# san-soucie/gdrf

Measured on AMD Instinct MI355X. Metric: ELBO steps/sec (+ achieved HBM GB/s on K_nm) at N=1e6,M=512,K=10,V=50, higher is better.
Workload: dtype f32; 1 GPU; configs[3] at 1 GPU(s): N=1000000 synthetic 2-D lattice (1000x1000), V=50, K=10, M=512 (32x16 grid inducing points), rbf kernel, Adam lr=1e-3, Trace_ELBO, 1 particle, jitter=1e-06, observations sharded over ranks; N=1000000, M=512, K=10, V=50, D=2, rows_per_rank=1000000, jitter_level=2, stores_T=False, mfma_mode=f16x3

## Files before the change

### gdrf_amd/csrc/api.hip

```cpp
#include "../../include/gdrf_hip.h"
#include "common.h"
#include "gemm_nt.h"
#include "gemm_tn.h"
#include "gemm_split.h"
#include "gemm_tn_topics.h"
#include "gemm_tn_topics1.h"
#include "kernels_mm.h"
#include "kernels_n.h"
#include "predict.h"
#include "predict_mc.h"
#include "predict_info.h"
#include "foldin.h"
#include "sample_counts.h"
#include "predict_cov.h"
#include "select_batch.h"
#include "rows_lds.h"
#include "rows_mfma.h"
#include "rows_vstream.h"
#include "rows_csr.h"
#include "hyper_tn.h"
#include "optim.h"

#include <algorithm>
#include <cmath>
// ... 831 lines not shown
        constexpr int lds4 = 8 * SplitCfg<SP>::IMG * 2 + 8 * GDRF_TILE * 4;
        HIPCHK(hipFuncSetAttribute((const void*)fwd_t_split_q4_kernel<SP>, hipFuncAttributeMaxDynamicSharedMemorySize, lds4));
        hipLaunchKernelGGL(fwd_t_split_q4_kernel<SP>, dim3((unsigned)(8 * K * rt8)), dim3(1024), lds4, s, a);
      } else {
        constexpr int lds2 = 6 * SplitCfg<SP>::IMG * 2;
        HIPCHK(hipFuncSetAttribute((const void*)fwd_t_split_cc_kernel<SP>, hipFuncAttributeMaxDynamicSharedMemorySize, lds2));
        hipLaunchKernelGGL(fwd_t_split_cc_kernel<SP>, dim3((unsigned)(8 * K * rt8)), dim3(512), lds2, s, a);
      }
      LAUNCHCHK("fwd_t_split");
      return 0;
    } else {
      return fail(-1, "fwd_t_split", "float arrays only");
    }
  }

  template <class SP>
  static int tn_split(gdrf_ctx* c, const float* B, const float* scale, int64_t scale_bs, int64_t n, int64_t rps, int sym, float* slab,
                      int nbatch, int ns, int ntiles, int sidx_b, int sidx_b_stride, hipStream_t s, const void* Ah = nullptr, int sidx_a = -1) {
    if constexpr (std::is_same<T, float>::value) {
      using E = typename SP::E;
      TNSplitArgs<SP> a{(const E*)(Ah ? Ah : c->Wh), (int64_t)c->ncap * c->Mp, c->Mp, B, c->Mp, scale, scale_bs, n, rps, c->Mp, sym, slab, nbatch, ns,
                        (const float*)c->ssc, sidx_a >= 0 ? sidx_a : SplitLay{c->K}.w(), sidx_b, sidx_b_stride};
      constexpr int lds = 3 * SP::NP * 32 * 128 * 2;
      HIPCHK(hipFuncSetAttribute((const void*)gemm_tn_split_kernel<SP>, hipFuncAttributeMaxDynamicSharedMemorySize, lds));
      hipLaunchKernelGGL(gemm_tn_split_kernel<SP>, dim3((unsigned)(ntiles * nbatch * ns)), dim3(256), lds, s, a);
      return 0;
    } else {
      return fail(-1, "tn_split", "float arrays only");
    }
  }

  template <class SP>
  static int wbar_split(gdrf_ctx* c, int64_t n, const T* U, int64_t rtiles, hipStream_t s) {
    if constexpr (std::is_same<T, float>::value) {
      using E = typename SP::E;
      const int Mp = c->Mp, K = c->K;
      const SplitLay SL{K};
      const int64_t nb = (int64_t)K * Mp * Mp;
      hipLaunchKernelGGL(split_blocked_kernel<SP>, dim3((unsigned)((nb / 4 + 255) / 256)), dim3(256), 0, s, (const float*)c->Bm, nb, Mp, Mp, (E*)c->Bh, nb,
                         (const float*)c->ssc + SL.b(0));
      BwdWbarSplitArgs<SP> a{(const float*)c->W, (const E*)c->Wh, (int64_t)c->ncap * Mp, n, c->M, Mp, K, (const E*)c->Bh, nb,
                             (const float*)c->vbar, (const float*)c->locbar, c->ldk, (const float*)c->asum, (const float*)U, (float*)c->Wbar,
                             (const float*)c->ssc, c->smx + SL.mx_wbar()};
      const size_t grp = SplitCfg<SP>::LDS_BYTES + (((size_t)K * GDRF_TILE * sizeof(float) + 15) & ~(size_t)15);
      const int nct_ = (Mp + GDRF_TILE - 1) / GDRF_TILE;
      if (K >= 2 && 2 * grp <= 160 * 1024) {
        const int64_t pairs = (rtiles + 1) / 2;
        const size_t tabb = ((size_t)K * GDRF_TILE * sizeof(float) + 15) & ~(size_t)15;
        const size_t lds_cc = 6 * (size_t)SplitCfg<SP>::IMG * 2 + 2 * tabb;
        if (std::is_same<SP, SplitF16>::value && K >= 2 && (Mp % 64) == 0 && 8 * (size_t)SplitCfg<SP>::IMG * 2 + 2 * tabb <= 160 * 1024) {
          if constexpr (std::is_same<SP, SplitF16>::value) {
            const size_t lds64 = 8 * (size_t)SplitCfg<SP>::IMG * 2 + 2 * tabb;
            const int nkb = Mp / 64;
            int nslice = 1;
            if (pairs * nct_ <= 32 && nkb >= 2) nslice = std::min(nkb, 8);
            if ((size_t)nslice * round_up(n, 256) * Mp > (size_t)c->nsplit_cap * (K + 1) * Mp * Mp) nslice = 1;
            if (nslice > 1) { a.slab = (float*)c->slab; a.slab_stride = (int64_t)round_up(n, 256) * Mp; a.nslice = nslice; }
            c->forms[GDRF_FORM_WBAR] = 6; c->forms[GDRF_FORM_WBAR_NSLICE] = nslice;
            HIPCHK(hipFuncSetAttribute((const void*)bwd_wbar_f16_k64_kernel, hipFuncAttributeMaxDynamicSharedMemorySize, (int)lds64));
            hipLaunchKernelGGL(bwd_wbar_f16_k64_kernel, dim3((unsigned)round_up(pairs * nct_, 8), (unsigned)nslice), dim3(512), lds64, s, a);
            if (nslice > 1) {
              const int64_t n4 = n * Mp / 4;
              hipLaunchKernelGGL(wbar_slab_sum_kernel, dim3((unsigned)((n4 + 255) / 256)), dim3(256), 0, s, (const float*)a.slab, a.slab_stride, nslice, n4,
                                 (float*)c->Wbar, a.wbar_max);
            }
          }
        } else if (lds_cc <= 160 * 1024) {
          HIPCHK(hipFuncSetAttribute((const void*)bwd_wbar_split_cc_kernel<SP>, hipFuncAttributeMaxDynamicSharedMemorySize, (int)lds_cc));
          hipLaunchKernelGGL((bwd_wbar_split_cc_kernel<SP>), dim3((unsigned)round_up(pairs * nct_, 8)), dim3(512), lds_cc, s, a);
          c->forms[GDRF_FORM_WBAR] = 5; c->forms[GDRF_FORM_WBAR_NSLICE] = 1;
        } else {
          const size_t lds = std::max<size_t>(2 * grp, 8 * 32 * 68 * sizeof(float));
          HIPCHK(hipFuncSetAttribute((const void*)bwd_wbar_split_kernel<SP, 2>, hipFuncAttributeMaxDynamicSharedMemorySize, (int)lds));
          hipLaunchKernelGGL((bwd_wbar_split_kernel<SP, 2>), dim3((unsigned)round_up(pairs * nct_, 8)), dim3(512), lds, s, a);
          c->forms[GDRF_FORM_WBAR] = 4; c->forms[GDRF_FORM_WBAR_NSLICE] = 1;
        }
      } else {
        if (grp > 160 * 1024) return fail(-1, "wbar_split", "too many topics for the LDS scale table");
        const size_t lds = std::max<size_t>(grp, 4 * 32 * 68 * sizeof(float));
        HIPCHK(hipFuncSetAttribute((const void*)bwd_wbar_split_kernel<SP, 1>, hipFuncAttributeMaxDynamicSharedMemorySize, (int)lds));
        hipLaunchKernelGGL((bwd_wbar_split_kernel<SP, 1>), dim3((unsigned)round_up(rtiles * nct_, 8)), dim3(256), lds, s, a);
        c->forms[GDRF_FORM_WBAR] = 3; c->forms[GDRF_FORM_WBAR_NSLICE] = 1;
      }
      LAUNCHCHK("wbar_split");
      return 0;
    } else {
      return fail(-1, "wbar_split", "float arrays only");
    }
  }

  static int knm_solve(gdrf_ctx* c, const T* X, int64_t n, hipStream_t s) {
    ScopedTimer tm(c, 1, s);
    const int VE = Vec16<TS>::N;
    const int vpr = (c->Mp + VE - 1) / VE, rpp = vpr <= 256 ? 256 / vpr : 1;
    int64_t blocks = (n + 4 * rpp - 1) / (4 * rpp);
    const int64_t kcap = 256 * 64;
    if (blocks > kcap) blocks = kcap;
    if (blocks < 1) blocks = 1;
    if constexpr (sizeof(TS) == 8) {
      if (c->kind == 0 && vpr <= 256) {
        auto go = [&](auto kern) {
          hipLaunchKernelGGL(kern, dim3((unsigned)blocks), dim3(256), 0, s, X, n, (const double*)Q(c->Zs), c->M, c->D, c->hyp, (double*)Q(c->Knm),
                             (int64_t)c->Mp);
        };
        if (ard_fwd(c)) { if (c->D <= 2) go(knm_rbf_f64_kernel<T, 2, true, true>); else go(knm_rbf_f64_kernel<T, GDRF_DMAX, true, true>); }
        else { if (c->D <= 2) go(knm_rbf_f64_kernel<T, 2>); else go(knm_rbf_f64_kernel<T, GDRF_DMAX>); }
// ... 1377 lines not shown
```

### gdrf_amd/csrc/gemm_split.h

```cpp
#pragma once
#include "common.h"
#include "gemm_nt.h"
#include "kernels_mm.h"

namespace gdrf {

typedef __bf16 bf16x8 __attribute__((ext_vector_type(8)));
typedef __bf16 bf16x4 __attribute__((ext_vector_type(4)));
typedef _Float16 f16x8 __attribute__((ext_vector_type(8)));
typedef _Float16 f16x4 __attribute__((ext_vector_type(4)));
typedef float f32x4 __attribute__((ext_vector_type(4)));
typedef uint32_t u32x4 __attribute__((ext_vector_type(4)));

struct SplitBf16 {
  using E = __bf16; using V8 = bf16x8; using V4 = bf16x4;
  static constexpr int NP = 3, NPROD = 6, ID = 1;
  static __device__ __forceinline__ constexpr int pa(int t) { constexpr int v[6] = {0, 1, 2, 0, 1, 0}; return v[t]; }
  static __device__ __forceinline__ constexpr int pb(int t) { constexpr int v[6] = {2, 1, 0, 1, 0, 0}; return v[t]; }
  static __device__ __forceinline__ f32x4 mma(V8 a, V8 b, f32x4 c) { return __builtin_amdgcn_mfma_f32_16x16x32_bf16(a, b, c, 0, 0, 0); }
  static __device__ __forceinline__ void split(float x, E (&p)[NP]) {
    p[0] = (__bf16)x;
    const float r1 = x - (float)p[0];
    p[1] = (__bf16)r1;
    p[2] = (__bf16)(r1 - (float)p[1]);
  }
};
struct SplitF16 {
  using E = _Float16; using V8 = f16x8; using V4 = f16x4;
  static constexpr int NP = 2, NPROD = 3, ID = 2;
  static __device__ __forceinline__ constexpr int pa(int t) { constexpr int v[3] = {0, 1, 0}; return v[t]; }
  static __device__ __forceinline__ constexpr int pb(int t) { constexpr int v[3] = {1, 0, 0}; return v[t]; }
  static __device__ __forceinline__ f32x4 mma(V8 a, V8 b, f32x4 c) { return __builtin_amdgcn_mfma_f32_16x16x32_f16(a, b, c, 0, 0, 0); }
  static __device__ __forceinline__ void split(float y, E (&p)[NP]) {
    p[0] = (_Float16)y;
    p[1] = (_Float16)(y - (float)p[0]);
  }
};

struct SplitLay {
  int K;
  __host__ __device__ int w() const { return 0; }
  __host__ __device__ int wbar() const { return 2; }
  __host__ __device__ int b(int k) const { return 4 + 2 * k; }
  __host__ __device__ int st(int k) const { return 4 + 2 * K + 2 * k; }
  __host__ __device__ int v(int k) const { return 4 + 4 * K + 2 * k; }
  __host__ __device__ int dk() const { return 4 + 6 * K; }
  __host__ __device__ int nfloats() const { return 6 + 6 * K; }
  __host__ __device__ int mx_wbar() const { return 0; }
  __host__ __device__ int mx_b(int k) const { return 1 + k; }
  __host__ __device__ int mx_st(int k) const { return 1 + K + k; }
  __host__ __device__ int mx_v(int k) const { return 1 + 2 * K + k; }
  __host__ __device__ int nmax() const { return 1 + 3 * K; }
};
// ... 9 lines not shown
__global__ void split_scales_kernel(int f16, const Hyper* __restrict__ h, const unsigned* __restrict__ mx, float* __restrict__ sc, int K, int what) {
  const SplitLay L{K};
  auto put = [&](int idx, float s) { sc[idx] = s; sc[idx + 1] = 1.0f / s; };
  const int t = threadIdx.x;
  if ((what & SPLIT_SC_W) && t == 0)
    put(L.w(), f16 ? split_pow2_scale(sqrtf((float)h->var), 13) : 1.0f);
  if ((what & SPLIT_SC_W) && t == 0) put(L.dk(), f16 ? split_pow2_scale(0.75f * (float)h->var, 15) : 1.0f);
  if ((what & SPLIT_SC_WBAR) && t == 0) put(L.wbar(), f16 ? split_pow2_scale(__uint_as_float(mx[L.mx_wbar()]), 15) : 1.0f);
  for (int k = t; k < K; k += blockDim.x) {
    if (what & SPLIT_SC_BST) {
      put(L.b(k), f16 ? split_pow2_scale(__uint_as_float(mx[L.mx_b(k)]), 15) : 1.0f);
      put(L.st(k), f16 ? split_pow2_scale(__uint_as_float(mx[L.mx_st(k)]), 15) : 1.0f);
    }
    if (what & SPLIT_SC_V) put(L.v(k), f16 ? split_pow2_scale(__uint_as_float(mx[L.mx_v(k)]) * sqrtf((float)h->var), 13) : 1.0f);
  }
}
__device__ __forceinline__ void wave_max_publish(unsigned* mx, float m) {
#pragma unroll
  for (int o = 32; o > 0; o >>= 1) m = fmaxf(m, __shfl_xor(m, o, 64));
  if ((threadIdx.x & 63) == 0 && m > 0) atomicMax(mx, __float_as_uint(m));
}

__global__ __launch_bounds__(256) void absmax_batched_kernel(const float* __restrict__ x, int64_t n, int64_t ld, unsigned* __restrict__ mx) {
  const int b = blockIdx.y;
  float m = 0;
  const f32x4* p = reinterpret_cast<const f32x4*>(x + (int64_t)b * ld);
  for (int64_t i = (int64_t)blockIdx.x * blockDim.x + threadIdx.x; i < (n >> 2); i += (int64_t)gridDim.x * blockDim.x) {
    const f32x4 v = p[i];
    m = fmaxf(fmaxf(m, fmaxf(fabsf(v[0]), fabsf(v[1]))), fmaxf(fabsf(v[2]), fabsf(v[3])));
  }
  if (blockIdx.x == 0 && threadIdx.x < (n & 3)) m = fmaxf(m, fabsf(x[(int64_t)b * ld + (n & ~(int64_t)3) + threadIdx.x]));
  wave_max_publish(mx + b, m);
}

template <class SP> struct SplitCfg {
  static constexpr int BK = 32;
  static constexpr int LDH = BK;
  static constexpr int PIECE = GDRF_TILE * LDH;
  static constexpr int IMG = SP::NP * PIECE;
  static constexpr int LDS_BYTES = 2 * IMG * 2;
};
__device__ __forceinline__ int split_swz(int row) { return (row & 8) ? 3 : 0; }
__device__ __forceinline__ int split_off(int row, int k) { return row * 32 + (((k >> 3) ^ split_swz(row)) << 3) + (k & 7); }

__device__ __forceinline__ void glds16_asm(const void* gsrc, unsigned lds_dst) {
  asm volatile("s_mov_b32 m0, %1\n\ts_nop 0\n\tglobal_load_lds_dwordx4 %0, off" : : "v"(gsrc), "s"(lds_dst) : "memory");
}
__device__ __forceinline__ void glds16_asm_s(const void* sbase, unsigned voff, unsigned lds_dst) {
  asm volatile("s_mov_b32 m0, %2\n\ts_nop 0\n\tglobal_load_lds_dwordx4 %0, %1" : : "v"(voff), "s"(sbase), "s"(lds_dst) : "memory");
}
__device__ __forceinline__ unsigned lds_addr(const void* p) {
  return (unsigned)(uintptr_t)(__attribute__((address_space(3))) const void*)p;
}


struct SplitLane {
  int tid, lane, wave;
  int wr, wc;
  int lr, lg;
  __device__ __forceinline__ SplitLane() {
    tid = threadIdx.x & 255; lane = tid & 63; wave = tid >> 6;
    wr = wave >> 1; wc = wave & 1; lr = lane & 15; lg = lane >> 4;
  }
  __device__ __forceinline__ int wave_u() const { return __builtin_amdgcn_readfirstlane(wave); }
  __device__ __forceinline__ int frag() const { return lr * 32 + ((lg ^ split_swz(lr)) << 3); }
  __device__ __forceinline__ int drow() const { return lane >> 2; }
  __device__ __forceinline__ int dq() const { return ((lane & 3) ^ split_swz(drow())) * 8; }
};

__device__ __forceinline__ void split_zero(f32x4 (&acc)[4][4]) {
#pragma unroll
  for (int a = 0; a < 4; ++a)
#pragma unroll
    for (int b = 0; b < 4; ++b) acc[a][b] = f32x4{0, 0, 0, 0};
}
template <class SP> __device__ __forceinline__ typename SP::V8 split_frag(const typename SP::E* img, int p, int row0, int frag) {
  return *reinterpret_cast<const typename SP::V8*>(img + p * SplitCfg<SP>::PIECE + row0 * 32 + frag);
}
template <class SP> __device__ __forceinline__ void split_frags(typename SP::V8 (&f)[SP::NP], const typename SP::E* img, int row0, int frag) {
#pragma unroll
  for (int p = 0; p < SP::NP; ++p) f[p] = split_frag<SP>(img, p, row0, frag);
}
template <class SP, bool FIRST>
__device__ __forceinline__ void split_products(f32x4 (&P)[4], const typename SP::V8 (&fa)[4][SP::NP], const typename SP::V8 (&fb)[SP::NP]) {
#pragma unroll
  for (int t = 0; t < SP::NPROD; ++t)
#pragma unroll
    for (int a = 0; a < 4; ++a) P[a] = SP::mma(fa[a][SP::pa(t)], fb[SP::pb(t)], (FIRST && t == 0) ? f32x4{0, 0, 0, 0} : P[a]);
}
__device__ __forceinline__ void split_row_scales(f32x4 (&s4)[4], const float* sc_row, const SplitLane& L) {
#pragma unroll
  for (int a = 0; a < 4; ++a) s4[a] = *reinterpret_cast<const f32x4*>(sc_row + L.wr * 64 + a * 16 + L.lg * 4);
}
__device__ __forceinline__ void split_scaled_acc(f32x4 (&acc)[4][4], int b, const f32x4 (&s4)[4], const f32x4 (&P)[4]) {
#pragma unroll
  for (int a = 0; a < 4; ++a)
#pragma unroll
    for (int r = 0; r < 4; ++r) acc[a][b][r] += s4[a][r] * P[a][r];
}
__device__ __forceinline__ void split_phase_end() {
  asm volatile("s_waitcnt vmcnt(0)" ::: "memory");
  asm volatile("s_waitcnt lgkmcnt(0)" ::: "memory");
  gdrf_raw_barrier();
}


// ... 465 lines not shown
      const int64_t mc = m < g.nrows ? m : 0;
      const int nc = n < Mp ? n : 0;
      wv[h][i] = *reinterpret_cast<const f32x4*>(g.W + mc * Mp + nc);
      as2v[h][i] = first_slice ? 2.0f * g.asum[mc] : 0.0f;
    }
  const int wr = L.wr, wc = L.wc, lr = L.lr, lg = L.lg;
  for (int kb = 0; kb < (first_slice ? K : 0); kb += 16) {
    float av[4][4], bv[4][4];
#pragma unroll
    for (int it = 0; it < 4; ++it) {
      const int k = kb + 4 * it + lg, kc = k < K ? k : 0;
#pragma unroll
      for (int a = 0; a < 4; ++a) {
        const int64_t row = m0 + wr * 64 + a * 16 + lr;
        const float v = g.locbar[(int64_t)kc * g.ldk + (row < g.nrows ? row : 0)];
        av[it][a] = (k < K && row < g.nrows) ? v : 0.0f;
      }
#pragma unroll
      for (int b = 0; b < 4; ++b) {
        const int col = n0 + wc * 64 + b * 16 + lr;
        const float v = g.U[(int64_t)kc * g.M + (col < g.M ? col : 0)];
        bv[it][b] = (k < K && col < g.M) ? v : 0.0f;
      }
    }
#pragma unroll
    for (int it = 0; it < 4; ++it) {
      if (kb + 4 * it < K) {
#pragma unroll
        for (int a = 0; a < 4; ++a)
#pragma unroll
          for (int b = 0; b < 4; ++b) acc[a][b] = __builtin_amdgcn_mfma_f32_16x16x4f32(av[it][a], bv[it][b], acc[a][b], 0, 0, 0);
      }
    }
  }
  __syncthreads();
  float wmax = 0.0f;
  float* tile = wbar_tile(smem, gp, L);
#pragma unroll
  for (int h = 0; h < 2; ++h) {
    wbar_tile_put(tile, acc, h, L);
#pragma unroll
    for (int i = 0; i < 8; ++i) {
      const int64_t m = m0 + L.wr * 64 + h * 32 + ((L.lane >> 4) + 4 * i);
      const int n = n0 + L.wc * 64 + (L.lane & 15) * 4;
      const f32x4 t = wbar_tile_get(tile, i, L);
      if (m < g.nrows && n < Mp) wbar_seg_store(out_base + m * Mp + n, t, as2v[h][i], wv[h][i], wmax);
    }
    asm volatile("s_waitcnt lgkmcnt(0)" ::: "memory");
  }
  if (g.wbar_max && g.nslice == 1) wave_max_publish(g.wbar_max, wmax);
}


__global__ __launch_bounds__(256) void wbar_slab_sum_kernel(const float* __restrict__ slab, int64_t slab_stride, int nslice, int64_t n4 ,
                                                           float* __restrict__ Wbar, unsigned* __restrict__ wbar_max) {
  const int64_t i = (int64_t)blockIdx.x * blockDim.x + threadIdx.x;
  float wmax = 0.0f;
  if (i < n4) {
    f32x4 acc = *reinterpret_cast<const f32x4*>(slab + 4 * i);
    for (int sl = 1; sl < nslice; ++sl) {
      const f32x4 t = *reinterpret_cast<const f32x4*>(slab + (int64_t)sl * slab_stride + 4 * i);
#pragma unroll
      for (int e = 0; e < 4; ++e) acc[e] += t[e];
    }
    *reinterpret_cast<f32x4*>(Wbar + 4 * i) = acc;
#pragma unroll
    for (int e = 0; e < 4; ++e) wmax = fmaxf(wmax, fabsf(acc[e]));
  }
  if (wbar_max) wave_max_publish(wbar_max, wmax);
}

template <class SP> struct FwdTSplitArgs {
  const typename SP::E* Wh; int64_t w_stride; int64_t nrows; int Mp, K;
  int KG; int rt8;
  const typename SP::E* STh; int64_t piece_stride;
  float* tt; int64_t ldt;
  const float* sc;
};

template <class SP> __device__ __forceinline__ void fwd_t_map_block(const FwdTSplitArgs<SP>& g, int64_t& rt0, int& bz) {
  const unsigned xcd = blockIdx.x & 7u, idx = blockIdx.x >> 3;
  const unsigned per_group = (unsigned)g.KG * (unsigned)g.rt8;
  const int grp = (int)(idx / per_group);
  const unsigned rem = idx - (unsigned)grp * per_group;
  const int kg = min(g.KG, g.K - grp * g.KG);
  rt0 = 2 * ((int64_t)(rem / (unsigned)kg) * 8 + xcd);
  bz = grp * g.KG + (int)(rem % (unsigned)kg);
}
__device__ __forceinline__ bool fwd_t_col_ok(int ct, int b, int Mp, const SplitLane& L) { return ct * GDRF_TILE + L.wc * 64 + b * 16 + L.lr < Mp; }
__device__ __forceinline__ float fwd_t_sq(float x, bool cok) { return cok ? x * x : 0.0f; }
template <class SP> __device__ __forceinline__ void fwd_t_store_tt(const FwdTSplitArgs<SP>& g, int bz, int64_t m0, int tid, float v) {
  const int64_t m = m0 + tid;
  const SplitLay SL{g.K};
  const float un = g.sc[SL.w() + 1] * g.sc[SL.st(bz) + 1];
  if (m < g.nrows) g.tt[(int64_t)bz * g.ldt + m] = v * (un * un);
}


template <class SP>
__global__ __launch_bounds__(512, 2) void fwd_t_split_cc_kernel(FwdTSplitArgs<SP> g) {
  using CF = SplitCfg<SP>;
  using E = typename SP::E;
  using V8 = typename SP::V8;
  constexpr int NP = SP::NP;
  extern __shared__ __attribute__((aligned(16))) char smem[];
  constexpr int IMG = CF::IMG;
// ... 422 lines not shown
```

### gdrf_amd/csrc/gemm_tn_topics1.h

```cpp
#pragma once
#include <utility>
#include "gemm_tn_topics.h"

namespace gdrf {

template <int... Is, class F> __device__ __forceinline__ void static_for_impl(std::integer_sequence<int, Is...>, F&& f) {
  (f(std::integral_constant<int, Is>{}), ...);
}
template <int N, class F> __device__ __forceinline__ void static_for(F&& f) { static_for_impl(std::make_integer_sequence<int, N>{}, f); }

constexpr int TN1_CH = 64;
constexpr int TN1_XBLK = 1056;
constexpr int TN1_X_BYTES = 16 * TN1_XBLK;
constexpr int TN1_VROWS = 12;
constexpr int TN1_V_BYTES = TN1_VROWS * TN1_CH * 4;
constexpr int TN1_NBUF = 3;

__device__ __forceinline__ void glds4_asm(const void* gsrc, unsigned lds_dst) {
  asm volatile("s_mov_b32 m0, %1\n\ts_nop 0\n\tglobal_load_lds_dword %0, off" : : "v"(gsrc), "s"(lds_dst) : "memory");
}

__device__ __forceinline__ void glds4_asm_s(const void* sbase, unsigned voff, unsigned lds_dst) {
  asm volatile("s_mov_b32 m0, %2\n\ts_nop 0\n\tglobal_load_lds_dword %0, %1" : : "v"(voff), "s"(sbase), "s"(lds_dst) : "memory");
}

__global__ void tn1_scale_rows_kernel(const float* __restrict__ vbar, int64_t ldk, int64_t nrows, float* __restrict__ vs, int64_t lds,
                                      const float* __restrict__ sc, int sidx_v) {
  const int k = blockIdx.y;
  const float scale = sc[sidx_v + 2 * k];
  for (int64_t n = (int64_t)blockIdx.x * blockDim.x + threadIdx.x; n < lds; n += (int64_t)gridDim.x * blockDim.x)
    vs[(int64_t)k * lds + n] = n < nrows ? vbar[(int64_t)k * ldk + n] * scale : 0.0f;
}

constexpr int TN2_A_BYTES = 2 * 2 * 32 * 128 * 2;
constexpr int TN2_BUF = TN2_A_BYTES + TN1_X_BYTES + TN1_V_BYTES;
constexpr int TN2_DMA_PER_CHUNK = 15;
constexpr int tn2_lds_bytes() { return TN1_NBUF * TN2_BUF; }

__host__ __device__ inline int tn2_ntiles_half(int ncols) {
  const int nI = (ncols + 127) / 128, nJ = (ncols + 63) / 64;
  int t = 0;
  for (int I = 0; I < nI; ++I) t += (2 * I + 1 < nJ) ? 1 : 0;
  return t;
}
template <int AMIN>
__global__ __launch_bounds__(256, 1) void tn_topics_w2_kernel(TNTopicsArgs g) {
  using E = _Float16;
  using V8 = f16x8;
  using V4 = f16x4;
  constexpr int KT = TNT_KT, PIECE = 32 * 128, KA = 8;
  static_assert(KT == 10, "register plan below is for 10 topics");
  extern __shared__ __attribute__((aligned(16))) char smem[];
  const int tid = threadIdx.x, lane = tid & 63;
  const int w = __builtin_amdgcn_readfirstlane(tid >> 6);
  const int lr = lane & 15, lg = lane >> 4;
  const int kgroups = (g.K + KT - 1) / KT;
  const unsigned units = (unsigned)(g.ntiles * kgroups), bid = blockIdx.x;
  unsigned u; int sp;
  if ((g.nsplit & 7) == 0) { const unsigned idx = bid >> 3; sp = (int)(idx / units) * 8 + (int)(bid & 7u); u = idx % units; }
  else { sp = (int)(bid / units); u = bid % units; }
  const int tile = (int)(u % (unsigned)g.ntiles), gk = (int)(u / (unsigned)g.ntiles);
  int I = 0, J = tile;
// ... 217 lines not shown
```

### gdrf_amd/engine.py

```python
from __future__ import annotations

import contextlib
import ctypes as C
import math
from typing import Dict, Optional

import torch

from . import _lib
from .data import check_counts, is_sparse_counts

KERNEL_IDS = {"rbf": 0, "matern52": 1, "matern32": 2, "exponential": 3, "rationalquadratic": 4, "periodic": 5, "product": 6}
PRODUCT_KINDS = {"rbf": 0, "periodic": 5}
OPT_MODES = {"adam": 0, "adamw": 1, "clippedadam": 2}
OPT_RULES = {"adam": 0, "adamw": 1, "clippedadam": 2, "adamax": 3, "rmsprop": 4, "adagrad": 5, "adadelta": 6, "asgd": 7, "rprop": 8,
             "adagradrmsprop": 9}
OPT_CLIP_NORM, OPT_CLIP_VALUE, OPT_MOMENTUM, OPT_CENTERED = 1, 2, 4, 8

_WS_IDS = dict(W=0, Wbar=1, q=2, loc=3, tt=4, vbar=5, locbar=6, asum=7, Kuu=8, L=9, Linv=10, S=11, B=12, phi=13,
               mu=14, LinvT=15, ST=16, Knm=17, g_locbar=18)


def _stream_ptr(device) -> int:
    return torch.cuda.current_stream(device).cuda_stream
# ... 362 lines not shown
            fi = torch.finfo(self.dtype)
            y = self.Z.clamp(min=fi.tiny, max=1.0 - fi.eps)
            self.view("inducing_unc").copy_(y.log() - (-y).log1p())

    def refresh_inducing(self):
        if self.learn_inducing:
            torch.sigmoid(self.view("inducing_unc"), out=self.Z)

    def set_dirichlet(self, alpha: torch.Tensor):
        a = alpha.detach().to("cpu", torch.float64).contiguous()
        assert a.shape == (self.K, self.V)
        arr = (C.c_double * (self.K * self.V))(*a.flatten().tolist())
        _lib.check(self.lib.gdrf_set_dirichlet(self.ctx, arr), "gdrf_set_dirichlet")

    def workspace(self, name: str, n_rows: Optional[int] = None) -> torch.Tensor:
        ptr, cnt = C.c_void_p(), C.c_int64()
        _lib.check(self.lib.gdrf_ws_ptr(self.ctx, _WS_IDS[name], C.byref(ptr), C.byref(cnt)), "gdrf_ws_ptr")
        esz = self.lib.gdrf_ws_elem_size(self.ctx, _WS_IDS[name])
        flat = torch.empty(cnt.value, dtype=torch.float32 if esz == 4 else torch.float64, device=self.device)
        _lib.check(self.lib.gdrf_ws_copy(self.ctx, _WS_IDS[name], flat.data_ptr(), cnt.value, _stream_ptr(self.device)),
                   "gdrf_ws_copy")
        torch.cuda.synchronize(self.device)
        Mp = (self.M + 31) // 32 * 32
        ldk = (self.n_cap + 3) // 4 * 4
        n = self.n_cap if n_rows is None else n_rows
        if name in ("W", "Wbar", "Knm"):
            return flat.view(self.n_cap, Mp)[:n, :self.M].clone()
        if name in ("q", "asum"):
            return flat[:n].clone()
        if name in ("loc", "tt", "vbar", "locbar", "mu"):
            return flat.view(self.K, ldk)[:, :n].clone()
        if name in ("Kuu", "L", "Linv", "LinvT"):
            return flat.view(Mp, Mp)[:self.M, :self.M].clone()
        if name in ("S", "B", "ST"):
            return flat.view(self.K, Mp, Mp)[:, :self.M, :self.M].clone()
        if name == "phi":
            return flat.view(self.K, self.V).clone()
        raise KeyError(name)

    TIMING_SLOTS = ("probe", "k_nm", "transforms", "fwd_w", "loc", "fwd_t", "elbo_rows", "bwd_wbar", "bwd_knm",
                    "tn_sym", "tn_gt", "slab_reduce", "ubar", "step_finish", "adam", "factorize")

    def set_timing(self, enable: bool):
        _lib.check(self.lib.gdrf_set_timing(self.ctx, 1 if enable else 0), "gdrf_set_timing")

    def get_timing(self) -> Dict[str, Dict[str, float]]:
        n = len(self.TIMING_SLOTS)
        ms, cnt = (C.c_double * n)(), (C.c_int64 * n)()
        _lib.check(self.lib.gdrf_get_timing(self.ctx, ms, cnt, n), "gdrf_get_timing")
        return {name: dict(ms=ms[i], count=cnt[i]) for i, name in enumerate(self.TIMING_SLOTS)}

    FORM_SLOTS = ("wbar", "wbar_nslice", "a_k", "a_k_kgroups", "fwd_t", "fwd_t_kg", "loc", "ubar_q4", "rows", "rows_kt", "rows_vt", "gt",
                  "hyper", "predict", "predict_nb")
    FORM_NAMES = dict(wbar=("gemm_nt", "gemm_nt_t", "split<1>", "split<2>", "split_cc", "k64"), a_k=("gemm_tn", "tn_split", "tn_topics", "w2"),
                      fwd_t=("gemm_nt", "q4", "cc"), loc=("rows", "gemm_nt", "gemm_nt_wide"), rows=("mfma", "thread", "streamed"),
                      gt=("gemm_tn", "tn_split"), hyper=("f64", "tn"), predict=("mfma", "rows_lds", "rows_mem", "rows_bigk", "streamed"))

    def last_forms(self) -> Dict[str, object]:
        n = len(self.FORM_SLOTS)
        arr = (C.c_int * n)()
        _lib.check(self.lib.gdrf_last_forms(self.ctx, arr, n), "gdrf_last_forms")
        out = {}
        for slot, v in zip(self.FORM_SLOTS, arr):
            if v:
                out[slot] = self.FORM_NAMES[slot][v - 1] if slot in self.FORM_NAMES else v
        return out

    def _chk_rows(self, xs: torch.Tensor, ws: Optional[torch.Tensor] = None):
        if xs.device != self.device or xs.dtype != self.dtype or not xs.is_contiguous() or xs.dim() != 2 or xs.shape[1] != self.D:
            raise ValueError(f"xs must be a contiguous ({'n'},{self.D}) {self.dtype} tensor on {self.device}")
        if ws is not None and is_sparse_counts(ws):
            check_counts(ws, xs.shape[0], self.V, self.device)
        elif ws is not None:
            if ws.device != self.device or ws.dtype != torch.int32 or not ws.is_contiguous() or ws.shape != (xs.shape[0], self.V):
                raise ValueError(f"ws must be a contiguous (n,{self.V}) int32 tensor on {self.device}")

    def _counts_ptr(self, ws: Optional[torch.Tensor]):
        if ws is None or not is_sparse_counts(ws):
            if self._csr_bound:
                _lib.check(self.lib.gdrf_bind_counts_csr(self.ctx, None, None, None, 0, 0, None, None), "gdrf_bind_counts_csr")
                self._csr_bound = False
            return None if ws is None else ws.data_ptr()
        c = self._csr_cache
        if c is None or c[0] is not ws or c[1] != ws._version:
            crow = ws.crow_indices().to(torch.int64).contiguous()
            col = ws.col_indices().to(torch.int32).contiguous()
            val = ws.values().contiguous()
            order = torch.sort(col, stable=True)
            cperm = order.indices.to(torch.int64).contiguous()
            ccol = torch.searchsorted(order.values, torch.arange(self.V + 1, dtype=torch.int32, device=self.device)).to(torch.int64).contiguous()
            c = self._csr_cache = (ws, ws._version, (crow, col, val, ccol, cperm))
            self._csr_bound = False
        if not self._csr_bound:
            crow, col, val, ccol, cperm = c[2]
            _lib.check(self.lib.gdrf_bind_counts_csr(self.ctx, crow.data_ptr(), col.data_ptr(), val.data_ptr(), ws.shape[0], col.numel(),
                                                     ccol.data_ptr(), cperm.data_ptr()), "gdrf_bind_counts_csr")
            self._csr_bound = True
        return None

    def knm(self, xs: torch.Tensor) -> torch.Tensor:
        self._chk_rows(xs)
        out = torch.empty(xs.shape[0], self.M, dtype=self.dtype, device=self.device)
        self.knm_into(xs, out)
        return out

    def knm_into(self, xs: torch.Tensor, out: torch.Tensor):
        _lib.check(self.lib.gdrf_knm(self.ctx, xs.data_ptr(), xs.shape[0], self.Z.data_ptr(), self.params.data_ptr(),
# ... 519 lines not shown
```

Before: 24.37 steps/s.

## Add hand-scheduled AGPR-resident f16-split Wbar backward kernel for large row counts

Adds a new Wbar backward kernel, used when there are many row tiles and K is at most 16. It holds W fragments and B tiles in AGPRs through inline assembly and interleaves MFMA, global loads, LDS DMA and scale reads on a fixed static schedule. It uses one wave per column half, 256 threads and a single block per CU, and folds the rank-K locbar·U correction in afterwards with fp32 MFMA. The goal is to hide memory latency and raise MFMA utilization compared with the k64 kernel, at the cost of very fragile hand-tuned code: clobbering every AGPR, hard-coded vmcnt counts and low occupancy. The static_for helper moves into a shared header.

After: 24.85 steps/s (median of 6 runs). 1.02x the previous value.

```diff
diff --git a/gdrf_amd/csrc/api.hip b/gdrf_amd/csrc/api.hip
--- a/gdrf_amd/csrc/api.hip
+++ b/gdrf_amd/csrc/api.hip
@@ -907,6 +907,19 @@
           if constexpr (std::is_same<SP, SplitF16>::value) {
             const size_t lds64 = 8 * (size_t)SplitCfg<SP>::IMG * 2 + 2 * tabb;
             const int nkb = Mp / 64;
+            if (pairs * nct_ > 32 && K <= 16) {
+              const size_t lds_w1 = 8 * (size_t)SplitCfg<SP>::IMG * 2 + 2 * (size_t)(K + 1) * GDRF_TILE * sizeof(float);
+              const dim3 grid((unsigned)round_up(pairs * nct_, 8));
+              auto launch = [&](auto kern) {
+                HIPCHK(hipFuncSetAttribute((const void*)kern, hipFuncAttributeMaxDynamicSharedMemorySize, (int)lds_w1));
+                hipLaunchKernelGGL(kern, grid, dim3(256), lds_w1, s, a);
+                return 0;
+              };
+              if (int rc = K >= 8 ? launch(bwd_wbar_f16_w1_kernel<2>) : (K >= 4 ? launch(bwd_wbar_f16_w1_kernel<4>) : launch(bwd_wbar_f16_w1_kernel<8>))) return rc;
+              c->forms[GDRF_FORM_WBAR] = 7; c->forms[GDRF_FORM_WBAR_NSLICE] = 1;
+              LAUNCHCHK("wbar_split");
+              return 0;
+            }
             int nslice = 1;
             if (pairs * nct_ <= 32 && nkb >= 2) nslice = std::min(nkb, 8);
             if ((size_t)nslice * round_up(n, 256) * Mp > (size_t)c->nsplit_cap * (K + 1) * Mp * Mp) nslice = 1;
diff --git a/gdrf_amd/csrc/gemm_split.h b/gdrf_amd/csrc/gemm_split.h
--- a/gdrf_amd/csrc/gemm_split.h
+++ b/gdrf_amd/csrc/gemm_split.h
@@ -1,4 +1,5 @@
 #pragma once
+#include <utility>
 #include "common.h"
 #include "gemm_nt.h"
 #include "kernels_mm.h"
@@ -114,6 +115,11 @@
 __device__ __forceinline__ unsigned lds_addr(const void* p) {
   return (unsigned)(uintptr_t)(__attribute__((address_space(3))) const void*)p;
 }
+
+template <int... Is, class F> __device__ __forceinline__ void static_for_impl(std::integer_sequence<int, Is...>, F&& f) {
+  (f(std::integral_constant<int, Is>{}), ...);
+}
+template <int N, class F> __device__ __forceinline__ void static_for(F&& f) { static_for_impl(std::make_integer_sequence<int, N>{}, f); }
 
 
 struct SplitLane {
@@ -685,6 +691,255 @@
 }
 
 
+#define GDRF_A10(p) "a" p "0", "a" p "1", "a" p "2", "a" p "3", "a" p "4", "a" p "5", "a" p "6", "a" p "7", "a" p "8", "a" p "9"
+#define GDRF_A100(p) GDRF_A10(p "0"), GDRF_A10(p "1"), GDRF_A10(p "2"), GDRF_A10(p "3"), GDRF_A10(p "4"), GDRF_A10(p "5"), GDRF_A10(p "6"), \
+                     GDRF_A10(p "7"), GDRF_A10(p "8"), GDRF_A10(p "9")
+#define GDRF_ALL_AGPRS "a0", "a1", "a2", "a3", "a4", "a5", "a6", "a7", "a8", "a9", GDRF_A10("1"), GDRF_A10("2"), GDRF_A10("3"), GDRF_A10("4"), \
+                       GDRF_A10("5"), GDRF_A10("6"), GDRF_A10("7"), GDRF_A10("8"), GDRF_A10("9"), GDRF_A100("1"), GDRF_A10("20"), GDRF_A10("21"), \
+                       GDRF_A10("22"), GDRF_A10("23"), GDRF_A10("24"), "a250", "a251", "a252", "a253", "a254", "a255"
+constexpr int wb1_wreg(int ks, int a, int p) { return ((ks * 8 + a) * 2 + p) * 4; }
+constexpr int wb1_breg(int h, int ks, int b, int p) { return 128 + (((h * 2 + ks) * 4 + b) * 2 + p) * 4; }
+template <int WA, int BA, bool ZERO> __device__ __forceinline__ void wb1_mfma(f32x4& P) {
+  if constexpr (ZERO) asm volatile("v_mfma_f32_16x16x32_f16 %0, a[%c1:%c2], a[%c3:%c4], 0" : "=v"(P) : "i"(WA), "i"(WA + 3), "i"(BA), "i"(BA + 3));
+  else asm volatile("v_mfma_f32_16x16x32_f16 %0, a[%c1:%c2], a[%c3:%c4], %0" : "+v"(P) : "i"(WA), "i"(WA + 3), "i"(BA), "i"(BA + 3));
+}
+template <int REG, int OFF> __device__ __forceinline__ void wb1_gload(const void* sbase, unsigned voff) {
+  asm volatile("global_load_dwordx4 a[%c2:%c3], %0, %1 offset:%c4" : : "v"(voff), "s"(sbase), "i"(REG), "i"(REG + 3), "i"(OFF) : "memory", GDRF_ALL_AGPRS);
+}
+template <int REG, int OFF> __device__ __forceinline__ void wb1_ldsread(unsigned addr) {
+  asm volatile("ds_read_b128 a[%c1:%c2], %0 offset:%c3" : : "v"(addr), "i"(REG), "i"(REG + 3), "i"(OFF) : "memory", GDRF_ALL_AGPRS);
+}
+template <int R0> __device__ __forceinline__ void wb1_update2(float& c0, float& c1, const f32x4& s, const f32x4& p) {
+  asm volatile("v_fmac_f32 %0, %1, %2" : "+v"(c0) : "v"(s[R0]), "v"(p[R0]));
+  asm volatile("v_fmac_f32 %0, %1, %2" : "+v"(c1) : "v"(s[R0 + 1]), "v"(p[R0 + 1]));
+}
+template <int N> __device__ __forceinline__ void wb1_vmcnt() { asm volatile("s_waitcnt vmcnt(%0)" : : "n"(N) : "memory"); }
+
+template <int R>
+__global__ __launch_bounds__(256, 1) void bwd_wbar_f16_w1_kernel(BwdWbarSplitArgs<SplitF16> g) {
+  using SP = SplitF16;
+  using CF = SplitCfg<SP>;
+  using E = typename SP::E;
+  static_assert(R == 2 || R == 4 || R == 8, "16 requests per block in K >= 16 / R phases");
+  constexpr int PIECE = CF::PIECE;
+  constexpr int WIMG = 4 * PIECE * 2;
+  extern __shared__ __attribute__((aligned(16))) char smem[];
+  SplitLane L;
+  const int w = L.wave_u(), gp = w >> 1, wc = w & 1;
+  L.wc = wc;
+  const int K = g.K, Mp = g.Mp;
+  const int tabf = (K + 1) * GDRF_TILE;
+  float* const tab0 = reinterpret_cast<float*>(smem + 4 * WIMG);
+  const int nct = (Mp + GDRF_TILE - 1) / GDRF_TILE;
+  int64_t rtile; int ct;
+  nt_xcd_map_paired(blockIdx.x, nct, gp, rtile, ct);
+  const int64_t m0 = rtile * GDRF_TILE;
+  const int n0 = ct * GDRF_TILE;
+  wbar_fill_scales(g, tab0, (rtile - gp) * GDRF_TILE, L.tid);
+  wbar_fill_scales(g, tab0 + tabf, (rtile - gp + 1) * GDRF_TILE, L.tid);
+  tab0[(L.tid >> 7) * tabf + K * GDRF_TILE + (L.tid & 127)] = 0.0f;
+  const float* const tab = tab0 + gp * tabf;
+
+  const int nk = Mp / 64, nph = nk * K;
+  const int lr = L.lr, lg = L.lg, drow = L.drow(), dq = L.dq();
+  const unsigned w_lds = lds_addr(smem) + (unsigned)(gp * WIMG);
+  const unsigned frag_addr = w_lds + (unsigned)(L.frag() * 2);
+  const int64_t mbase = m0 < g.nrows ? m0 : 0;
+  auto w_off = [&](int i) {
+    const int64_t rel = (wc + 2 * i) * 16 + drow, last = g.nrows - 1 - mbase;
+    unsigned v = (unsigned)(((int)(rel < last ? rel : last) * Mp + dq) * 2);
+    asm volatile("" : "+v"(v));
+    return v;
+  };
+  const unsigned vw0 = w_off(0), vw1 = w_off(1), vw2 = w_off(2), vw3 = w_off(3);
+  const E* const w_row = g.Wh + mbase * Mp;
+  auto dma_w = [&](int q, int buf, int rep_c, auto jc) {
+    constexpr int j = decltype(jc)::value;
+    const int r = rep_c * R + j, ks = r >> 3, p = (r >> 2) & 1;
+    const unsigned va = (j & 1) ? vw1 : vw0, vb = (j & 1) ? vw3 : vw2;
+    const unsigned vo = R >= 4 ? ((j & 2) ? vb : va) : ((rep_c & 1) ? vb : va);
+    const int rbk = wc + 2 * (r & 3);
+    const E* src = w_row + (p ? g.w_stride : 0) + q * 64 + ks * 32;
+    const unsigned dst = w_lds + (unsigned)(buf * 2 * WIMG + (ks * 2 + p) * PIECE * 2 + rbk * 1024);
+    asm volatile("s_mov_b32 m0, %2\n\ts_nop 4\n\tglobal_load_lds_dwordx4 %0, %1" : : "v"(vo), "s"(src), "s"(dst) : "memory");
+  };
+  const int col0 = (n0 + wc * 64 < Mp) ? n0 + wc * 64 : 0;
+  const unsigned voff_b = (unsigned)((lr * 32 + 8 * lg) * 2);
+  const int64_t b_ks = (int64_t)Mp * 32, b_rep = (int64_t)(Mp >> 5) * b_ks;
+  const E* sb[2][2];
+  auto b_bases = [&](const E* b0) {
+    sb[0][0] = b0; sb[1][0] = b0 + b_ks; sb[0][1] = b0 + g.piece_stride; sb[1][1] = b0 + b_ks + g.piece_stride;
+#pragma unroll
+    for (int i = 0; i < 4; ++i) asm volatile("" : "+s"(sb[i >> 1][i & 1]));
+  };
+  const E* b_blk = g.Bh + (int64_t)col0 * 32;
+  const E* b_cur = b_blk;
+
+  float acc[8][4][4];
+  f32x4 P[8], s8[8];
+#pragma unroll
+  for (int a = 0; a < 8; ++a) {
+    P[a] = f32x4{0, 0, 0, 0}; s8[a] = f32x4{0, 0, 0, 0};
+#pragma unroll
+    for (int b = 0; b < 4; ++b)
+#pragma unroll
+      for (int r = 0; r < 4; ++r) acc[a][b][r] = 0.0f;
+  }
+  for (int rp = 0; rp < 16 / R; ++rp) static_for<R>([&](auto jc) { dma_w(0, 0, rp, jc); });
+  b_bases(b_cur);
+  static_for<16>([&](auto jc) {
+    constexpr int j = decltype(jc)::value, bb = j >> 2, ks = (j >> 1) & 1, p = j & 1;
+    wb1_gload<wb1_breg(0, ks, bb, p), bb * 1024>(sb[ks][p], voff_b);
+  });
+  wb1_vmcnt<0>();
+  __syncthreads();
+
+  constexpr int N1 = R / 2, N2 = R / 2;
+  int c = 0, q = 0, rep = 0;
+  for (int it = 0; it < (nph + 1) / 2; ++it) {
+    static_for<2>([&](auto hc) {
+      constexpr int h = decltype(hc)::value;
+      const bool live = c < nph;
+      const int qq = q < nk ? q : nk - 1;
+      if (live && rep == 0) {
+        if (c > 0) { wb1_vmcnt<0>(); gdrf_raw_barrier(); }
+        const unsigned fa = frag_addr + (unsigned)((qq & 1) * 2 * WIMG);
+        static_for<32>([&](auto fc) {
+          constexpr int f = decltype(fc)::value, ks = f >> 4, p = (f >> 3) & 1, a = f & 7;
+          wb1_ldsread<wb1_wreg(ks, a, p), ((ks * 2 + p) * PIECE + a * 16 * 32) * 2>(fa);
+        });
+        asm volatile("s_waitcnt lgkmcnt(0)" ::: "memory");
+      }
+      const unsigned saddr = lds_addr(tab + (live ? rep : K) * GDRF_TILE + lg * 4);
+      const E* const b_next = c + 1 >= nph ? b_cur : (rep + 1 == K ? b_blk + 2 * b_ks : b_cur + b_rep);
+      b_bases(b_next);
+      const int qn = qq + 1 < nk ? qq + 1 : nk - 1, bufn = (qq + 1) & 1;
+      const int rep_c = (live && rep < 16 / R) ? rep : 16 / R - 1;
+      static_for<4>([&](auto bc) {
+        constexpr int b = decltype(bc)::value;
+        wb1_vmcnt<b == 0 ? 12 + N1 + N2 : (b == 1 ? 16 + 2 * N1 + N2 : (b == 2 ? 20 + N1 + N2 : 16 + N1 + 2 * N2))>();
+        static_for<48>([&](auto mc) {
+          constexpr int m = decltype(mc)::value, half = m / 24, mm = m % 24, ks = mm / 12, t = (mm >> 2) % 3, a = half * 4 + (mm & 3);
+          wb1_mfma<wb1_wreg(ks, a, SP::pa(t)), wb1_breg(h, ks, b, SP::pb(t)), mm < 4>(P[a]);
+          if constexpr (mm >= 4 && mm < 12) {
+            constexpr int i = mm - 4, au = (half == 0 ? 4 : 0) + (i >> 1), bu = half == 0 ? (b + 3) & 3 : b;
+            wb1_update2<2 * (i & 1)>(acc[au][bu][2 * (i & 1)], acc[au][bu][2 * (i & 1) + 1], s8[au], P[au]);
+          }
+          if constexpr (b == 0) {
+            if constexpr (m < 4) asm volatile("ds_read_b128 %0, %1 offset:%c2" : "=v"(s8[m]) : "v"(saddr), "i"(m * 64) : "memory");
+            if constexpr (m >= 13 && m < 20 && (m & 1)) asm volatile("ds_read_b128 %0, %1 offset:%c2" : "=v"(s8[4 + (m - 13) / 2]) : "v"(saddr), "i"((4 + (m - 13) / 2) * 64) : "memory");
+            if constexpr (m == 27) asm volatile("s_waitcnt lgkmcnt(0)" : "+v"(s8[0]), "+v"(s8[1]), "+v"(s8[2]), "+v"(s8[3]), "+v"(s8[4]), "+v"(s8[5]), "+v"(s8[6]), "+v"(s8[7]) : : "memory");
+          }
+          if constexpr (b < 2 && m >= 12 && m < 28 && (m & 1) == 0) {
+            constexpr int j = 8 * b + (m - 12) / 2, bb = j >> 2, ks2 = (j >> 1) & 1, p2 = j & 1;
+            wb1_gload<wb1_breg(1 - h, ks2, bb, p2), bb * 1024>(sb[ks2][p2], voff_b);
+          }
+          if constexpr ((b == 0 || b == 2) && m >= 38 && m < 38 + 2 * N1 && (m & 1) == 0)
+            dma_w(qn, bufn, rep_c, std::integral_constant<int, (b == 0 ? 0 : N1) + (m - 38) / 2>{});
+        });
+      });
+      ++c;
+      b_cur = b_next;
+      if (++rep == K) { rep = 0; ++q; b_blk += 2 * b_ks; }
+    });
+  }
+  wb1_vmcnt<0>();
+  asm volatile("s_nop 15\n\ts_nop 15" : "+v"(P[4]), "+v"(P[5]), "+v"(P[6]), "+v"(P[7]));
+  static_for<8>([&](auto ic) {
+    constexpr int i = decltype(ic)::value;
+    wb1_update2<2 * (i & 1)>(acc[4 + (i >> 1)][3][2 * (i & 1)], acc[4 + (i >> 1)][3][2 * (i & 1) + 1], s8[4 + (i >> 1)], P[4 + (i >> 1)]);
+  });
+  f32x4 accv[2][4][4];
+#pragma unroll
+  for (int a = 0; a < 8; ++a)
+#pragma unroll
+    for (int b = 0; b < 4; ++b) accv[a >> 2][a & 3][b] = f32x4{acc[a][b][0], acc[a][b][1], acc[a][b][2], acc[a][b][3]};
+
+  L.lane = (int)__builtin_amdgcn_mbcnt_hi(~0u, __builtin_amdgcn_mbcnt_lo(~0u, 0u));
+  L.lr = L.lane & 15; L.lg = L.lane >> 4;
+  f32x4 wv[2][2][8];
+  float as2v[2][2][8];
+  auto load_w = [&](int hr) {
+    L.wr = hr;
+#pragma unroll
+    for (int h = 0; h < 2; ++h)
+#pragma unroll
+      for (int i = 0; i < 8; ++i) {
+        const int64_t m = m0 + wbar_seg_row(L, h, i);
+        const int n = n0 + wbar_seg_col(L);
+        wv[hr][h][i] = *reinterpret_cast<const f32x4*>(g.W + (m < g.nrows ? m : 0) * Mp + (n < Mp ? n : 0));
+      }
+  };
+  load_w(0);
+#pragma unroll
+  for (int hr = 0; hr < 2; ++hr) {
+    L.wr = hr;
+#pragma unroll
+    for (int h = 0; h < 2; ++h)
+#pragma unroll
+      for (int i = 0; i < 8; ++i) {
+        const int64_t m = m0 + wbar_seg_row(L, h, i);
+        as2v[hr][h][i] = 2.0f * g.asum[m < g.nrows ? m : 0];
+      }
+  }
+  for (int kb = 0; kb < K; kb += 8) {
+    float av[2][8], bv[2][4];
+#pragma unroll
+    for (int it = 0; it < 2; ++it) {
+      const int k = kb + 4 * it + L.lg, kc = k < K ? k : 0;
+#pragma unroll
+      for (int a = 0; a < 8; ++a) {
+        const int64_t row = m0 + a * 16 + L.lr;
+        const float v = g.locbar[(int64_t)kc * g.ldk + (row < g.nrows ? row : 0)];
+        av[it][a] = (k < K && row < g.nrows) ? v : 0.0f;
+      }
+#pragma unroll
+      for (int b = 0; b < 4; ++b) {
+        const int col = n0 + wc * 64 + b * 16 + L.lr;
+        const float v = g.U[(int64_t)kc * g.M + (col < g.M ? col : 0)];
+        bv[it][b] = (k < K && col < g.M) ? v : 0.0f;
+      }
+    }
+#pragma unroll
+    for (int it = 0; it < 2; ++it) {
+      if (kb + 4 * it < K) {
+#pragma unroll
+        for (int a = 0; a < 8; ++a)
+#pragma unroll
+          for (int b = 0; b < 4; ++b)
+            asm volatile("s_nop 1\n\tv_mfma_f32_16x16x4_f32 %0, %1, %2, %0" : "+v"(accv[a >> 2][a & 3][b]) : "v"(av[it][a]), "v"(bv[it][b]));
+      }
+    }
+  }
+#pragma unroll
+  for (int hr = 0; hr < 2; ++hr)
+#pragma unroll
+    for (int a = 0; a < 4; ++a)
+      asm volatile("s_nop 15" : "+v"(accv[hr][a][0]), "+v"(accv[hr][a][1]), "+v"(accv[hr][a][2]), "+v"(accv[hr][a][3]));
+  __syncthreads();
+  float wmax = 0.0f;
+  L.wave = w;
+  float* tile = wbar_tile(smem, 0, L);
+#pragma unroll
+  for (int hr = 0; hr < 2; ++hr) {
+    L.wr = hr;
+#pragma unroll
+    for (int h = 0; h < 2; ++h) {
+      wbar_tile_put(tile, accv[hr], h, L);
+      if (hr == 0 && h == 1) { load_w(1); L.wr = 0; }
+#pragma unroll
+      for (int i = 0; i < 8; ++i) {
+        const int64_t m = m0 + wbar_seg_row(L, h, i);
+        const int n = n0 + wbar_seg_col(L);
+        const f32x4 t = wbar_tile_get(tile, i, L);
+        if (m < g.nrows && n < Mp) wbar_seg_store(g.Wbar + m * Mp + n, t, as2v[hr][h][i], wv[hr][h][i], wmax);
+      }
+      asm volatile("s_waitcnt lgkmcnt(0)" ::: "memory");
+    }
+  }
+  if (g.wbar_max) wave_max_publish(g.wbar_max, wmax);
+}
+
 __global__ __launch_bounds__(256) void wbar_slab_sum_kernel(const float* __restrict__ slab, int64_t slab_stride, int nslice, int64_t n4 ,
                                                            float* __restrict__ Wbar, unsigned* __restrict__ wbar_max) {
   const int64_t i = (int64_t)blockIdx.x * blockDim.x + threadIdx.x;
diff --git a/gdrf_amd/csrc/gemm_tn_topics1.h b/gdrf_amd/csrc/gemm_tn_topics1.h
--- a/gdrf_amd/csrc/gemm_tn_topics1.h
+++ b/gdrf_amd/csrc/gemm_tn_topics1.h
@@ -1,13 +1,7 @@
 #pragma once
-#include <utility>
 #include "gemm_tn_topics.h"
 
 namespace gdrf {
-
-template <int... Is, class F> __device__ __forceinline__ void static_for_impl(std::integer_sequence<int, Is...>, F&& f) {
-  (f(std::integral_constant<int, Is>{}), ...);
-}
-template <int N, class F> __device__ __forceinline__ void static_for(F&& f) { static_for_impl(std::make_integer_sequence<int, N>{}, f); }
 
 constexpr int TN1_CH = 64;
 constexpr int TN1_XBLK = 1056;
diff --git a/gdrf_amd/engine.py b/gdrf_amd/engine.py
--- a/gdrf_amd/engine.py
+++ b/gdrf_amd/engine.py
@@ -438,7 +438,7 @@
 
     FORM_SLOTS = ("wbar", "wbar_nslice", "a_k", "a_k_kgroups", "fwd_t", "fwd_t_kg", "loc", "ubar_q4", "rows", "rows_kt", "rows_vt", "gt",
                   "hyper", "predict", "predict_nb")
-    FORM_NAMES = dict(wbar=("gemm_nt", "gemm_nt_t", "split<1>", "split<2>", "split_cc", "k64"), a_k=("gemm_tn", "tn_split", "tn_topics", "w2"),
+    FORM_NAMES = dict(wbar=("gemm_nt", "gemm_nt_t", "split<1>", "split<2>", "split_cc", "k64", "w1"), a_k=("gemm_tn", "tn_split", "tn_topics", "w2"),
                       fwd_t=("gemm_nt", "q4", "cc"), loc=("rows", "gemm_nt", "gemm_nt_wide"), rows=("mfma", "thread", "streamed"),
                       gt=("gemm_tn", "tn_split"), hyper=("f64", "tn"), predict=("mfma", "rows_lds", "rows_mem", "rows_bigk", "streamed"))
 
```
